# ouyangjiahong/representation-disentanglement

Measured on AMD Instinct MI355X. Metric: MR slices/sec (train step, recon+adv+latent losses), higher is better.
Workload: dtype f32

## Files before the change

### include/mrdis.h

```cpp
#ifndef MRDIS_H
#define MRDIS_H

#include <stddef.h>
#include <stdint.h>

#ifdef __cplusplus
extern "C" {
#endif

#define MRDIS_OK            0
#define MRDIS_EINVAL       -1
#define MRDIS_EUNSUPPORTED -2
#define MRDIS_EWORKSPACE   -3
#define MRDIS_ELAUNCH      -4
#define MRDIS_EALIGN       -5

#define MRDIS_MAX_TAPS 16

#define MRDIS_EPI_NONE   0
#define MRDIS_EPI_LRELU  1

const char* mrdis_strerror(int code);
int mrdis_version(void);

// ... 110 lines not shown
                                 void* dx, int lddx, void* dgamma, int lddg, void* dbeta, int lddb,
                                 void* workspace, size_t workspace_bytes,
                                 int N, int Hi, int Wi, int C, const void* xlo, int ldxlo, int dtype, void* stream);

int mrdis_bilinear_fwd(const void* x, int ldx, void* y, int ldy, int N, int Hi, int Wi,
                       int Ho, int Wo, int C, int align_corners, int dtype, void* stream);
size_t mrdis_bilinear_up2_stats_workspace(int N, int Hi, int C);
int mrdis_bilinear_up2_stats_applies(int N, int Wi, int C);
int mrdis_bilinear_up2_stats_fwd(const void* x, int ldx, void* y, int ldy, int N, int Hi, int Wi, int C,
                                 int out_block, long long out_block_stride,
                                 float* save_mean, float* save_rstd, float eps, void* workspace, size_t workspace_bytes,
                                 int dtype, void* stream);
int mrdis_bilinear_bwd(const void* dy, int lddy, void* dx, int lddx, int N, int Hi, int Wi,
                       int Ho, int Wo, int C, int align_corners, int dtype, void* stream);

int mrdis_softmax_mask_drop_fwd(const float* s, int lds, const float* mask_img, float* out, int ldo,
                                long long P, int C, float mask_scale, void* stream);
int mrdis_softmax_mask_drop_bwd(const float* dout, int lddo, const float* out, int ldo,
                                float* ds, int ldds, long long P, int C, void* stream);

size_t mrdis_recon_err_workspace(int N, long long HW, int C);
int mrdis_recon_err_fwd(const float* gt, int ldgt, const float* x, int ldx, float* out,
                        void* workspace, size_t workspace_bytes,
                        int N, long long HW, int C, int p, void* stream);
int mrdis_recon_err_bwd(const float* gt, int ldgt, const float* x, int ldx, const float* w,
                        float* dx, int lddx, int N, long long HW, int C, int p, void* stream);

size_t mrdis_recon_metrics_workspace(int n_img, int H);
int mrdis_recon_metrics(const float* target, int ldt, const float* pred, int ldp, float* out,
                        void* workspace, size_t workspace_bytes, int n_img, int H, int W, void* stream);
// ... 146 lines not shown
```

### representation-disentanglement_amd/csrc/mrdis_common.h

```cpp
#pragma once
#include <hip/hip_runtime.h>
#include <stdint.h>
#include "../../include/mrdis.h"
#include "mrdis_device.h"

#define MRDIS_CHECK_LAUNCH()                                     \
    do {                                                         \
        hipError_t e_ = hipGetLastError();                       \
        if (e_ != hipSuccess) return MRDIS_ELAUNCH;              \
    } while (0)

#define MRDIS_OPTIONS(X) \
    X(WINO, "wino", "MRDIS_WINO", 0, 1)  \
    X(NT_MB, "nt_mb", "MRDIS_NT_MB", 0, 128)  \
    X(WINO_PIPE, "wino_pipe", "MRDIS_WINO_PIPE", 0, 1)  \
    X(WINO_U, "wino_u", "MRDIS_WINO_U", 0, 1)  \
    X(WINO4, "wino4", "MRDIS_WINO4", 0, 1)  \
    X(WINO4R, "wino4r", "MRDIS_WINO4R", 0, 1)  \
    X(BCONV4, "bconv4", "MRDIS_BCONV4", 0, 1)  \
    X(SPLIT6, "split6", "MRDIS_SPLIT6", 0, 1)  \
    X(NO16, "debug_no16", "MRDIS_DEBUG_NO16", 1, 0) \
    X(NOTHIN, "debug_nothin", "MRDIS_DEBUG_NOTHIN", 1, 0) \
    X(NOC4, "debug_noc4", "MRDIS_DEBUG_NOC4", 1, 0) \
    X(NODMA, "debug_nodma", "MRDIS_DEBUG_NODMA", 1, 0) \
// ... 28 lines not shown
    X(CHATT, "chatt") X(SYMDIFF, "symdiff") X(RGATE, "rgate")  \
    X(DIRECT3D, "direct3d") X(C3D16, "c3d16") X(WGRAD3D, "wgrad3d") X(WGRAD3D16, "wgrad3d16") X(WINO_WGRAD3D, "wino_wgrad3d")  \
    X(VOLGATHER, "volgather")  \
    X(LOSS3D, "loss3d") X(SEGCOUNTS, "segcounts")  \
    X(SEGACCUM, "segaccum") X(SEGLABELS, "seglabels")  \
    X(SYNTHACCUM, "synthaccum") X(SYNTHFINISH, "synthfinish")  \
    X(SEG2DLABELS, "seg2dlabels") X(SEG2DFINISH, "seg2dfinish")  \
    X(FUSE, "fuse")  \
    X(REGSURF, "regsurf") X(EDT, "edt") X(SURFHIST, "surfhist")  \
    X(CCLABEL, "cclabel") X(CCCLEAN, "ccclean")  \
    X(STAT_VEC, "stat_vec") X(STAT_SCALAR, "stat_scalar") X(STAT_INTERP, "stat_interp")  \
    X(SPADE_UP2_ONEPASS, "spade_up2_onepass") X(SPADE_UP2_TWOPASS, "spade_up2_twopass")  \
    X(BIL_FWD_X2, "bil_fwd_x2") X(BIL_FWD_GENERAL, "bil_fwd_general")  \
    X(BIL_BWD_X2, "bil_bwd_x2") X(BIL_BWD_TIGHT3, "bil_bwd_tight3") X(BIL_BWD_TIGHT5, "bil_bwd_tight5") X(BIL_BWD_GENERAL, "bil_bwd_general")  \
    X(ELEM_V1, "elem_v1")  \
    X(ALL, "all")
#define MRDIS_X_CNT_ID(id, name) MRDIS_CNT_##id,
enum { MRDIS_COUNTERS(MRDIS_X_CNT_ID) MRDIS_CNT_COUNT };
void mrdis_count(int id);

void mrdis_note_lds(const char* kernel_expr, size_t bytes);
#define MRDIS_LAUNCH(kernel, grid, block, lds, s, ...) do { mrdis_count(MRDIS_CNT_ALL); if ((size_t)(lds) != 0) mrdis_note_lds(#kernel, (size_t)(lds)); hipLaunchKernelGGL(kernel, grid, block, lds, s, __VA_ARGS__); } while (0)

int mrdis_cu_count();
bool mrdis_lds_optin(const void* kernel, int bytes);
int mrdis_occupancy(const void* kernel, int block, size_t lds);

static inline int mrdis_cdiv(long long a, long long b) { return (int)((a + b - 1) / b); }

__device__ __forceinline__ int mrdis_xcd_remap(int bid, int nblk) {
// ... 19 lines not shown
```

### representation-disentanglement_amd/csrc/mrdis_elem.hip

```cpp
#include "mrdis_common.h"
#include <type_traits>
#include <stdlib.h>

template <int V> struct Vec;
template <> struct Vec<1> {
    float v[1];
    __device__ __forceinline__ void load(const float* p) { v[0] = p[0]; }
    __device__ __forceinline__ void store(float* p) const { p[0] = v[0]; }
    __device__ __forceinline__ void load(const __bf16* p) { v[0] = (float)p[0]; }
    __device__ __forceinline__ void store(__bf16* p) const { p[0] = (__bf16)v[0]; }
};
template <> struct Vec<4> {
    float v[4];
    __device__ __forceinline__ void load(const float* p) {
        const float4 t = *reinterpret_cast<const float4*>(p); v[0] = t.x; v[1] = t.y; v[2] = t.z; v[3] = t.w;
    }
    __device__ __forceinline__ void store(float* p) const { *reinterpret_cast<float4*>(p) = make_float4(v[0], v[1], v[2], v[3]); }
    __device__ __forceinline__ void load(const __bf16* p) {
        const bf16x4 t = *reinterpret_cast<const bf16x4*>(p); v[0] = (float)t[0]; v[1] = (float)t[1]; v[2] = (float)t[2]; v[3] = (float)t[3];
    }
    __device__ __forceinline__ void store(__bf16* p) const {
        bf16x4 t; t[0] = (__bf16)v[0]; t[1] = (__bf16)v[1]; t[2] = (__bf16)v[2]; t[3] = (__bf16)v[3];
        *reinterpret_cast<bf16x4*>(p) = t;
    }
// ... 1120 lines not shown
        MRDIS_LAUNCH((bilinear_bwd_tight_kernel<4, 3, 3, T>), dim3(Hi, N), dim3(bil_threads((long long)Wi * (C / 4))), 0, s, dy, lddy, dx, lddx, N, Hi, Wi, Ho, Wo, C, align_corners, sh, sw);
    } else if (vec4_ok(dy, lddy, C) && vec4_ok(dx, lddx, C) && tight5) {
        mrdis_count(MRDIS_CNT_BIL_BWD_TIGHT5);
        MRDIS_LAUNCH((bilinear_bwd_tight_kernel<4, 5, 5, T>), dim3(Hi, N), dim3(bil_threads((long long)Wi * (C / 4))), 0, s, dy, lddy, dx, lddx, N, Hi, Wi, Ho, Wo, C, align_corners, sh, sw);
    } else if (vec4_ok(dy, lddy, C) && vec4_ok(dx, lddx, C)) {
        mrdis_count(MRDIS_CNT_BIL_BWD_GENERAL);
        MRDIS_LAUNCH((bilinear_bwd_kernel<4, T>), dim3(Hi, N), dim3(bil_threads((long long)Wi * (C / 4))), 0, s, dy, lddy, dx, lddx, N, Hi, Wi, Ho, Wo, C, align_corners, sh, sw);
    } else {
        mrdis_count(MRDIS_CNT_BIL_BWD_GENERAL); mrdis_count(MRDIS_CNT_ELEM_V1);
        MRDIS_LAUNCH((bilinear_bwd_kernel<1, T>), dim3(Hi, N), dim3(bil_threads((long long)Wi * C)), 0, s, dy, lddy, dx, lddx, N, Hi, Wi, Ho, Wo, C, align_corners, sh, sw);
    }
    MRDIS_CHECK_LAUNCH();
    return MRDIS_OK;
}

extern "C" size_t mrdis_bilinear_up2_stats_workspace(int N, int Hi, int C) { return sizeof(float) * 2 * (size_t)N * Hi * C + 64; }
template <typename T>
static int bilinear_up2_stats_impl(const T* x, int ldx, T* y, int ldy, int N, int Hi, int Wi, int C, int out_block, long long out_block_stride,
                                   float* save_mean, float* save_rstd, float eps, void* workspace, size_t workspace_bytes, void* stream) {
    if (!x || !y || !save_mean || !save_rstd || !workspace || N < 1 || Hi < 1 || Wi < 1 || C < 1 || ldx < C || ldy < C) return MRDIS_EINVAL;
    if (out_block <= 0 || out_block >= N) { out_block = 0x7fffffff; out_block_stride = 0; }
    else if (N % out_block != 0 || out_block_stride < 4LL * out_block * Hi * Wi * ldy || out_block_stride % 4 != 0) return MRDIS_EINVAL;
    if (workspace_bytes < mrdis_bilinear_up2_stats_workspace(N, Hi, C)) return MRDIS_EWORKSPACE;
    const int threads = bil_threads((long long)Wi * (C / 4));
    if (N > 65535 || C % 4 != 0 || !vec4_ok(x, ldx, C) || !vec4_ok(y, ldy, C) || threads % (C / 4) != 0) return MRDIS_EUNSUPPORTED;
    hipStream_t s = (hipStream_t)stream;
    float* part = reinterpret_cast<float*>(workspace);
    MRDIS_LAUNCH((bilinear_up2_fwd_kernel<T, true>), dim3(Hi, N), dim3(threads), 0, s, x, ldx, y, ldy, Hi, Wi, C, part, out_block, out_block_stride);
    MRDIS_CHECK_LAUNCH();
    MRDIS_LAUNCH((stat_final_kernel<0>), dim3(mrdis_cdiv(N * C, 64)), dim3(64, stat_final_lanes(Hi)), 0, s, part, Hi, C, N, 4LL * Hi * Wi, eps, 0.f,
// ... 70 lines not shown
                          lrelu_bwd_impl((cbf)dy, lddy, (cbf)y, ldy, (bf)dx, lddx, P, C, slope, stream));
}
extern "C" int mrdis_bilinear_fwd(const void* x, int ldx, void* y, int ldy, int N, int Hi, int Wi, int Ho, int Wo, int C, int align_corners, int dtype, void* stream) {
    return MRDIS_BY_DTYPE(dtype, bilinear_fwd_impl((const float*)x, ldx, (float*)y, ldy, N, Hi, Wi, Ho, Wo, C, align_corners, stream),
                          bilinear_fwd_impl((cbf)x, ldx, (bf)y, ldy, N, Hi, Wi, Ho, Wo, C, align_corners, stream));
}
extern "C" int mrdis_bilinear_up2_stats_fwd(const void* x, int ldx, void* y, int ldy, int N, int Hi, int Wi, int C, int out_block, long long out_block_stride,
                                            float* save_mean, float* save_rstd, float eps, void* workspace, size_t workspace_bytes, int dtype, void* stream) {
    return MRDIS_BY_DTYPE(dtype,
        bilinear_up2_stats_impl((const float*)x, ldx, (float*)y, ldy, N, Hi, Wi, C, out_block, out_block_stride, save_mean, save_rstd, eps, workspace, workspace_bytes, stream),
        bilinear_up2_stats_impl((cbf)x, ldx, (bf)y, ldy, N, Hi, Wi, C, out_block, out_block_stride, save_mean, save_rstd, eps, workspace, workspace_bytes, stream));
}
extern "C" int mrdis_bilinear_bwd(const void* dy, int lddy, void* dx, int lddx, int N, int Hi, int Wi, int Ho, int Wo, int C, int align_corners, int dtype, void* stream) {
    return MRDIS_BY_DTYPE(dtype, bilinear_bwd_impl((const float*)dy, lddy, (float*)dx, lddx, N, Hi, Wi, Ho, Wo, C, align_corners, stream),
                          bilinear_bwd_impl((cbf)dy, lddy, (bf)dx, lddx, N, Hi, Wi, Ho, Wo, C, align_corners, stream));
}

template <int V, typename TS, typename TD>
__global__ void cast_view_kernel(const TS* __restrict__ src, int lds_, int Cs, TD* __restrict__ dst, int ldd, int Cd, long long P) {
    const int Q = Cd / V;
    EW_LOOP(P * Q) {
        const long long r = idx / Q; const int c = (int)(idx - r * Q) * V;
        Vec<V> a;
        if (c + V <= Cs) a.load(src + r * lds_ + c);
        else {
#pragma unroll
            for (int k = 0; k < V; ++k) a.v[k] = (c + k < Cs) ? mrdis_ld1(src + r * lds_ + c + k) : 0.f;
        }
        a.store(dst + r * ldd + c);
    }
// ... 499 lines not shown
```

### representation-disentanglement_amd/hip.py

```python
import collections
import ctypes
import os

import torch

_HERE = os.path.dirname(os.path.abspath(__file__))
LIB_PATH = os.path.join(_HERE, 'csrc', 'libmrdis_hip.so')


class MrdisLibraryError(RuntimeError):
    pass


class MrdisError(RuntimeError):
    pass


_lib = None
_c = ctypes
_P, _I, _L, _F, _Z = _c.c_void_p, _c.c_int, _c.c_longlong, _c.c_float, _c.c_size_t

_SIGS = {
    'mrdis_strerror': (_c.c_char_p, [_I]),
    'mrdis_version': (_I, []),
# ... 32 lines not shown
    'mrdis_cast_view': (_I, [_P, _I, _I, _I, _P, _I, _I, _I, _L, _P]),
    'mrdis_conv2d_bwd_weight_workspace': (_Z, [_I] * 9),
    'mrdis_conv2d_bwd_weight': (_I, [_P, _I, _P, _I, _P, _P, _P, _Z] + [_I] * 11 + [_P]),
    'mrdis_lrelu_bwd': (_I, [_P, _I, _P, _I, _P, _I, _L, _I, _F, _I, _P]),
    'mrdis_norm_workspace': (_Z, [_I, _L, _I]),
    'mrdis_bn_train_fwd': (_I, [_P, _I, _P, _I, _P, _P, _P, _P, _P, _P, _P, _Z, _L, _I, _F, _F, _I, _I, _P]),
    'mrdis_bn_eval_fwd': (_I, [_P, _I, _P, _I, _P, _P, _P, _P, _L, _I, _F, _I, _P]),
    'mrdis_bn_train_bwd': (_I, [_P, _I, _P, _I, _P, _P, _P, _P, _I, _P, _P, _P, _P, _P, _Z, _L, _I, _I, _I, _P]),
    'mrdis_instnorm_spade_fwd': (_I, [_P, _I, _P, _I, _P, _I, _P, _I, _P, _P, _P, _Z, _I, _L, _I, _F, _I, _P]),
    'mrdis_instnorm_spade_bwd_workspace': (_Z, [_I, _L, _I]),
    'mrdis_instnorm_spade_bwd': (_I, [_P, _I, _P, _I, _P, _I, _P, _P, _P, _I, _P, _I, _P, _I, _P, _Z, _I, _L, _I, _I, _P]),
    'mrdis_instnorm_spade_bwd_up2_workspace': (_Z, [_I, _I, _I, _I, _I]),
    'mrdis_instnorm_spade_bwd_up2': (_I, [_P, _I, _P, _I, _P, _I, _P, _P, _P, _I, _P, _I, _P, _I, _P, _Z, _I, _I, _I, _I, _P, _I, _I, _P]),
    'mrdis_bilinear_fwd': (_I, [_P, _I, _P, _I] + [_I] * 8 + [_P]),
    'mrdis_bilinear_bwd': (_I, [_P, _I, _P, _I] + [_I] * 8 + [_P]),
    'mrdis_bilinear_up2_stats_workspace': (_Z, [_I, _I, _I]),
    'mrdis_bilinear_up2_stats_applies': (_I, [_I, _I, _I]),
    'mrdis_bilinear_up2_stats_fwd': (_I, [_P, _I, _P, _I, _I, _I, _I, _I, _I, _L, _P, _P, _F, _P, _Z, _I, _P]),
    'mrdis_softmax_mask_drop_fwd': (_I, [_P, _I, _P, _P, _I, _L, _I, _F, _P]),
    'mrdis_softmax_mask_drop_bwd': (_I, [_P, _I, _P, _I, _P, _I, _L, _I, _P]),
    'mrdis_recon_err_workspace': (_Z, [_I, _L, _I]),
    'mrdis_recon_err_fwd': (_I, [_P, _I, _P, _I, _P, _P, _Z, _I, _L, _I, _I, _P]),
    'mrdis_recon_err_bwd': (_I, [_P, _I, _P, _I, _P, _P, _I, _I, _L, _I, _I, _P]),
    'mrdis_recon_metrics_workspace': (_Z, [_I, _I]),
    'mrdis_recon_metrics': (_I, [_P, _I, _P, _I, _P, _P, _Z, _I, _I, _I, _P]),
    'mrdis_slice_gather': (_I, [_P, _P, _P, _P, _I, _P, _P, _I, _I, _I, _I, _I, _I, _P]),
    'mrdis_volume_gather': (_I, [_P, _I, _P, _P, _I, _I, _I, _I, _I, _I, _I, _I, _I, _I, _P]),
    'mrdis_nvnet_loss_workspace': (_Z, [_L, _L]),
    'mrdis_nvnet_loss_fwd': (_I, [_P, _P, _P, _P, _P, _I, _P, _P, _P, _P, _P, _I, _c.c_double, _P, _P, _P, _Z, _P]),
    'mrdis_nvnet_loss_bwd': (_I, [_P, _P, _P, _P, _P, _I, _P, _P, _P, _P, _P, _I, _c.c_double, _P, _P, _P, _P, _P]),
# ... 104 lines not shown
                                   'zsearch')
VARIANT_FAMILIES = ('conv2src', 'ana_act')
LATENT_FAMILIES = ('kl', 'avgpool')
OUTDEC_FAMILIES = ('chatt', 'symdiff', 'rgate')
CONV3D_FAMILIES = ('direct3d', 'c3d16', 'wgrad3d', 'wgrad3d16', 'wino_wgrad3d')
DATA_FAMILIES = ('volgather',)
LOSS3D_FAMILIES = ('loss3d', 'segcounts')
SEGVOL_FAMILIES = ('segaccum', 'seglabels')
SYNTH_FAMILIES = ('synthaccum', 'synthfinish')
SEG2D_FAMILIES = ('seg2dlabels', 'seg2dfinish')
FUSE_FAMILIES = ('fuse',)
SURFDIST_FAMILIES = ('regsurf', 'edt', 'surfhist')
CC_FAMILIES = ('cclabel', 'ccclean')
ELEM_FAMILIES = ('stat_vec', 'stat_scalar', 'stat_interp', 'spade_up2_onepass', 'spade_up2_twopass', 'bil_fwd_x2', 'bil_fwd_general',
                 'bil_bwd_x2', 'bil_bwd_tight3', 'bil_bwd_tight5', 'bil_bwd_general', 'elem_v1')
SYNTH_MAX_SRC = 8
SEG2D_MAX_SETS = 16
SEG2D_MAX_VIEWS = 2
SEG2D_FLIPS = {'': 0, 'h': 1, 'w': 2}
FUSE_MAX_SRC = 8
FUSE_METHODS = ('mean', 'max', 'mean-max-min')
EDT_FAR = 1 << 30
EDT_MAX_SRC = 8
EDT_MAX_EXTENT = 1024
SURF_MAX_REGIONS = 4
CC_MAX_EXTENT = 1024
CC_LABEL_LAUNCHES = 3
CC_CONNECTIVITIES = (6, 18, 26)


# ... 7 lines not shown
    import re
    buf = _c.create_string_buffer(16384)
    load().mrdis_dynamic_lds_table(buf, 16384)
    out = {}
    for line in buf.value.decode().splitlines():
        expr, _, b = line.rpartition('=')
        if not expr or not b.isdigit():
            continue
        name = re.sub(r'<.*', '', expr.strip().lstrip('(')).strip()
        out[name] = max(out.get(name, 0), int(b))
    return out


def launch_counts(reset=False, elem=False):
    lib = load()
    fams = WINO_FAMILIES + VARIANT_FAMILIES + LATENT_FAMILIES + OUTDEC_FAMILIES + CONV3D_FAMILIES + DATA_FAMILIES + LOSS3D_FAMILIES + SEGVOL_FAMILIES + SYNTH_FAMILIES + SEG2D_FAMILIES + FUSE_FAMILIES + SURFDIST_FAMILIES + CC_FAMILIES
    out ={f: int(lib.mrdis_launch_count(f.encode())) for f in fams + (ELEM_FAMILIES if elem else ())}
    if reset:
        lib.mrdis_launch_count_reset()
    return out


class option:

    def __init__(self, name, value):
        self.name, self.value = name, value

    def __enter__(self):
        self.prev = get_option(self.name)
        set_option(self.name, self.value)

# ... 714 lines not shown

def bilinear_bwd(dy, in_hw, align_corners, out=None):
    lib = load()
    dy, lddy = nhwc(dy)
    N, C, Ho, Wo = dy.shape
    Hi, Wi = in_hw
    if out is None:
        dx = empty_nhwc(N, C, Hi, Wi, dy.device, dy.dtype)
    else:
        dx, ldo = nhwc(out)
        assert dx.data_ptr() == out.data_ptr() and ldo == C and tuple(out.shape) == (N, C, Hi, Wi) and out.dtype == dy.dtype
    _chk(lib.mrdis_bilinear_bwd(_ptr(dy), lddy, _ptr(dx), C, N, Hi, Wi, Ho, Wo, C, 1 if align_corners else 0, _dt(dy), _stream()), 'bilinear_bwd')
    return dx


def softmax_mask_drop_fwd(s, mask_img, scale=100.0):
    lib = load()
    s, lds = nhwc(s)
    N, C, H, W = s.shape
    out = empty_nhwc(N, C, H, W, s.device)
    m = None if mask_img is None else mask_img.contiguous()
    _chk(lib.mrdis_softmax_mask_drop_fwd(_ptr(s), lds, _ptr(m), _ptr(out), C, N * H * W, C, scale, _stream()), 'softmax_mask_drop_fwd')
    return out


def softmax_mask_drop_bwd(dout, out):
    lib = load()
    dout, lddo = nhwc(dout); out, ldo = nhwc(out)
    N, C, H, W = out.shape
    ds = empty_nhwc(N, C, H, W, out.device)
# ... 898 lines not shown
```

### representation-disentanglement_amd/model.py

```python
import copy
import weakref

import numpy as np
import torch
import torch.nn as nn
import torch.nn.functional as F

from . import ops


def _pair(v):
    return (v, v) if isinstance(v, int) else tuple(v)


class _routing(nn.Module):

    def __init__(self, in_channels, num_experts):
        super().__init__()
        self.fc = nn.Linear(in_channels, num_experts)

    def forward(self, inputs_type):
        return torch.sigmoid(self.fc(inputs_type))


# ... 212 lines not shown
        return self.act(x)


class Act_Deconv_BN_Concat_New(nn.Module):

    def __init__(self, in_num_ch, out_num_ch, filter_size=3, stride=1, padding=1, activation='relu', upsample=True,
                 is_last=False, is_bn=True, is_cond=False):
        super().__init__()
        if not upsample:
            raise NotImplementedError('ConvTranspose2d variant is not on the path (model.py:2178)')
        self.is_bn, self.is_cond, self.is_last = is_bn, is_cond, is_last
        self.act = nn.ELU(inplace=True) if activation == 'elu' else nn.Sequential()
        self.conv = Conv2d(is_cond)(in_num_ch, out_num_ch, filter_size, stride, padding=padding)
        self.bn = BatchNorm2d(out_num_ch)

    def forward(self, x_down, x_up, inputs_type=None):
        x_up = self.act(x_up)
        x_up = ops.bilinear(x_up, (2 * x_up.shape[2], 2 * x_up.shape[3]), True)
        x_up = self.conv(x_up, inputs_type) if self.is_cond else self.conv(x_up)
        if self.is_last:
            return x_up
        if self.is_bn and self.training and x_up.is_cuda and ops.cat_elision() and x_down.dtype == x_up.dtype and isinstance(self.act, nn.Sequential) \
                and x_down.shape[0] == x_up.shape[0] and x_down.shape[2:] == x_up.shape[2:]:
            Cd, Cu = x_down.shape[1], x_up.shape[1]
            buf = getattr(x_down, '_mrdis_catbuf', None)
            if buf is not None and buf.shape[1] == Cd + Cu and buf.dtype == x_up.dtype:
                x_down._mrdis_catbuf = None
                x_up = self.bn(x_up, into=(buf, Cd))
                return ops.cat_join(x_down, x_up, buf)
        if self.is_bn:
            x_up = self.bn(x_up)
        return torch.cat([x_down, x_up], 1)


    def forward_grouped(self, x_down, x_up, types):
        G = len(types)
        x_up = self.act(x_up)
        x_up = ops.bilinear(x_up, (2 * x_up.shape[2], 2 * x_up.shape[3]), True)
        x_up = self.conv.forward_grouped(x_up, types)
        if self.is_last:
            return x_up
        if self.is_bn and self.training and x_up.is_cuda and ops.cat_elision() and x_down.dtype == x_up.dtype and isinstance(self.act, nn.Sequential) \
                and x_down.shape[0] == x_up.shape[0] and x_down.shape[2:] == x_up.shape[2:]:
            Cd, Cu = x_down.shape[1], x_up.shape[1]
            buf = getattr(x_down, '_mrdis_catbuf', None)
            if buf is not None and buf.shape[1] == Cd + Cu and buf.dtype == x_up.dtype:
                x_down._mrdis_catbuf = None
                x_up = self.bn(x_up, into=(buf, Cd), groups=G)
                return ops.cat_join(x_down, x_up, buf)
        if self.is_bn:
            x_up = self.bn(x_up, groups=G)
        return torch.cat([x_down, x_up], 1)
# ... 1132 lines not shown
```

### representation-disentanglement_amd/ops.py

```python
import contextlib
import numpy as _np
import os as _os

import torch
from torch.autograd import Function

from . import hip


class _MixExperts(Function):

    @staticmethod
    def forward(ctx, W, r):
        w_tck, w_tkc = hip.mix_experts_fwd(W, r)
        ctx.save_for_backward(W, r)
        ctx.mark_non_differentiable(w_tkc)
        return w_tck, w_tkc

    @staticmethod
    def backward(ctx, g_tck, _g_tkc):
        W, r = ctx.saved_tensors
        dW, dr = hip.mix_experts_bwd(g_tck, W, r)
        return dW, dr

# ... 970 lines not shown
    @staticmethod
    def forward(ctx, x, out_hw, align_corners):
        ctx.geom = (x.shape[2], x.shape[3], align_corners)
        return hip.bilinear_fwd(x, out_hw, align_corners)

    @staticmethod
    def backward(ctx, dy):
        Hi, Wi, ac = ctx.geom
        return hip.bilinear_bwd(dy, (Hi, Wi), ac), None, None


def bilinear(x, out_hw, align_corners):
    return _Bilinear.apply(x, tuple(out_hw), bool(align_corners))


class _BilinearUp2Stats(Function):

    @staticmethod
    def forward(ctx, x, eps):
        ctx.geom = (x.shape[2], x.shape[3])
        res = hip.bilinear_up2_stats(x, eps)
        if res is None:
            y = hip.bilinear_fwd(x, (2 * x.shape[2], 2 * x.shape[3]), False)
            mean = rstd = torch.empty(0, dtype=torch.float32, device=x.device)
        else:
            y, mean, rstd = res
        ctx.mark_non_differentiable(mean, rstd)
        return y, mean, rstd

    @staticmethod
# ... 749 lines not shown
```

Before: 253.3.

## Fold final 3x3 conv before bilinear upsample via 1x1 conv and tap-sum kernel

```diff
diff --git a/include/mrdis.h b/include/mrdis.h
--- a/include/mrdis.h
+++ b/include/mrdis.h
@@ -148,6 +148,11 @@
 int mrdis_bilinear_bwd(const void* dy, int lddy, void* dx, int lddx, int N, int Hi, int Wi,
                        int Ho, int Wo, int C, int align_corners, int dtype, void* stream);
 
+int mrdis_up2_tapsum_fwd(const float* M, int ldm, const float* bias, float* y, int ldy, int N, int h, int w, int Co, void* stream);
+size_t mrdis_up2_tapsum_bwd_workspace(int N, int h, int w, int Co);
+int mrdis_up2_tapsum_bwd(const float* dy, int lddy, float* G, int ldg, float* dbias, int accumulate_bias, void* workspace, size_t workspace_bytes,
+                         int N, int h, int w, int Co, void* stream);
+
 int mrdis_softmax_mask_drop_fwd(const float* s, int lds, const float* mask_img, float* out, int ldo,
                                 long long P, int C, float mask_scale, void* stream);
 int mrdis_softmax_mask_drop_bwd(const float* dout, int lddo, const float* out, int ldo,
diff --git a/representation-disentanglement_amd/csrc/mrdis_common.h b/representation-disentanglement_amd/csrc/mrdis_common.h
--- a/representation-disentanglement_amd/csrc/mrdis_common.h
+++ b/representation-disentanglement_amd/csrc/mrdis_common.h
@@ -66,6 +66,7 @@
     X(BIL_FWD_X2, "bil_fwd_x2") X(BIL_FWD_GENERAL, "bil_fwd_general")  \
     X(BIL_BWD_X2, "bil_bwd_x2") X(BIL_BWD_TIGHT3, "bil_bwd_tight3") X(BIL_BWD_TIGHT5, "bil_bwd_tight5") X(BIL_BWD_GENERAL, "bil_bwd_general")  \
     X(ELEM_V1, "elem_v1")  \
+    X(UP2TAPSUM, "up2tapsum")  \
     X(ALL, "all")
 #define MRDIS_X_CNT_ID(id, name) MRDIS_CNT_##id,
 enum { MRDIS_COUNTERS(MRDIS_X_CNT_ID) MRDIS_CNT_COUNT };
diff --git a/representation-disentanglement_amd/csrc/mrdis_elem.hip b/representation-disentanglement_amd/csrc/mrdis_elem.hip
--- a/representation-disentanglement_amd/csrc/mrdis_elem.hip
+++ b/representation-disentanglement_amd/csrc/mrdis_elem.hip
@@ -1158,6 +1158,306 @@
     return MRDIS_OK;
 }
 
+constexpr int HEAD_TH = 16, HEAD_TW = 64, HEAD_LH = HEAD_TH / 2 + 3, HEAD_LW = HEAD_TW / 2 + 3;
+template <int CO>
+__device__ __forceinline__ void head_lds_load(const float* p, float (&v)[CO]) {
+    if constexpr (CO == 4) { const float4 t = *reinterpret_cast<const float4*>(p); v[0] = t.x; v[1] = t.y; v[2] = t.z; v[3] = t.w; }
+    else {
+#pragma unroll
+        for (int o = 0; o < CO; ++o) v[o] = p[o];
+    }
+}
+template <int CO>
+__device__ __forceinline__ void head_lds_store(float* p, const float (&v)[CO]) {
+    if constexpr (CO == 4) *reinterpret_cast<float4*>(p) = make_float4(v[0], v[1], v[2], v[3]);
+    else {
+#pragma unroll
+        for (int o = 0; o < CO; ++o) p[o] = v[o];
+    }
+}
+template <int CO>
+__global__ __launch_bounds__(256) void up2_tapsum_fwd_kernel(const float* __restrict__ M, int ldm, const float* __restrict__ bias, float* __restrict__ y, int ldy,
+                                                             int h, int w, float sh, float sw, int vec_m, int vec_y) {
+    constexpr int C9 = 9 * CO;
+    extern __shared__ __attribute__((aligned(16))) float head_tile[];
+    const int Ho = 2 * h, Wo = 2 * w, n = blockIdx.z;
+    const int Y0 = blockIdx.y * HEAD_TH, X0 = blockIdx.x * HEAD_TW;
+    const int ya = Y0 > 0 ? Y0 - 1 : 0, yb = Y0 + HEAD_TH < Ho ? Y0 + HEAD_TH : Ho - 1;
+    const int xa = X0 > 0 ? X0 - 1 : 0, xb = X0 + HEAD_TW < Wo ? X0 + HEAD_TW : Wo - 1;
+    const int r0 = bil_axis(ya, sh, 1, h).i0, c0 = bil_axis(xa, sw, 1, w).i0;
+    int nr = bil_axis(yb, sh, 1, h).i1 - r0 + 1, nc = bil_axis(xb, sw, 1, w).i1 - c0 + 1;
+    if (nr > HEAD_LH) nr = HEAD_LH;
+    if (nc > HEAD_LW) nc = HEAD_LW;
+    const float* src = M + (((long long)n * h + r0) * w + c0) * ldm;
+    if (CO == 4 && vec_m) {
+        constexpr int Q = C9 / 4, RPW = (HEAD_LH + 3) / 4, IPR = (HEAD_LW * Q + 63) / 64;
+        const int wave = threadIdx.x >> 6, lane = threadIdx.x & 63;
+        float4 t[RPW][IPR];
+#pragma unroll
+        for (int a = 0; a < RPW; ++a)
+#pragma unroll
+            for (int k = 0; k < IPR; ++k) {
+                const int r = wave + 4 * a, it = lane + 64 * k;
+                const bool ok = r < nr && it < nc * Q;
+                const int rc = ok ? r : 0, pix = (ok ? it : 0) / Q, q = (ok ? it : 0) - pix * Q;
+                t[a][k] = mrdis_ld4(src + ((long long)rc * w + pix) * ldm + 4 * q);
+            }
+#pragma unroll
+        for (int a = 0; a < RPW; ++a)
+#pragma unroll
+            for (int k = 0; k < IPR; ++k) {
+                const int r = wave + 4 * a, it = lane + 64 * k;
+                if (r < nr && it < nc * Q) *reinterpret_cast<float4*>(head_tile + r * (HEAD_LW * C9) + 4 * it) = t[a][k];
+            }
+    } else {
+        for (int idx = threadIdx.x; idx < nr * nc * C9; idx += 256) {
+            const int pix = idx / C9, k = idx - pix * C9, r = pix / nc, c = pix - r * nc;
+            head_tile[(r * HEAD_LW + c) * C9 + k] = src[((long long)r * w + c) * ldm + k];
+        }
+    }
+    __syncthreads();
+    float b[CO];
+#pragma unroll
+    for (int o = 0; o < CO; ++o) b[o] = bias ? bias[o] : 0.f;
+    for (int p = threadIdx.x; p < HEAD_TH * HEAD_TW; p += 256) {
+        const int Y = Y0 + p / HEAD_TW, X = X0 + p % HEAD_TW;
+        if (Y >= Ho || X >= Wo) continue;
+        BilAxis ah[3], aw[3];
+        bool vh[3], vw[3];
+#pragma unroll
+        for (int k = 0; k < 3; ++k) {
+            const int yy = Y + k - 1, xx = X + k - 1;
+            vh[k] = yy >= 0 && yy < Ho; vw[k] = xx >= 0 && xx < Wo;
+            ah[k] = bil_axis(vh[k] ? yy : Y, sh, 1, h); aw[k] = bil_axis(vw[k] ? xx : X, sw, 1, w);
+            ah[k].i0 = min(ah[k].i0 - r0, HEAD_LH - 1) * (HEAD_LW * C9); ah[k].i1 = min(ah[k].i1 - r0, HEAD_LH - 1) * (HEAD_LW * C9);
+            aw[k].i0 = min(aw[k].i0 - c0, HEAD_LW - 1) * C9; aw[k].i1 = min(aw[k].i1 - c0, HEAD_LW - 1) * C9;
+        }
+        float acc[CO];
+#pragma unroll
+        for (int o = 0; o < CO; ++o) acc[o] = b[o];
+#pragma unroll
+        for (int kh = 0; kh < 3; ++kh)
+#pragma unroll
+            for (int kw = 0; kw < 3; ++kw) {
+                if (!(vh[kh] && vw[kw])) continue;
+                const float* t = head_tile + (kh * 3 + kw) * CO;
+                float p00[CO], p01[CO], p10[CO], p11[CO];
+                head_lds_load<CO>(t + ah[kh].i0 + aw[kw].i0, p00); head_lds_load<CO>(t + ah[kh].i0 + aw[kw].i1, p01);
+                head_lds_load<CO>(t + ah[kh].i1 + aw[kw].i0, p10); head_lds_load<CO>(t + ah[kh].i1 + aw[kw].i1, p11);
+#pragma unroll
+                for (int o = 0; o < CO; ++o)
+                    acc[o] += ah[kh].l0 * (aw[kw].l0 * p00[o] + aw[kw].l1 * p01[o]) + ah[kh].l1 * (aw[kw].l0 * p10[o] + aw[kw].l1 * p11[o]);
+            }
+        float* yo = y + (((long long)n * Ho + Y) * Wo + X) * ldy;
+        if (CO == 4 && vec_y) mrdis_st4(yo, make_float4(acc[0], acc[CO > 1 ? 1 : 0], acc[CO > 2 ? 2 : 0], acc[CO > 3 ? 3 : 0]));
+        else {
+#pragma unroll
+            for (int o = 0; o < CO; ++o) yo[o] = acc[o];
+        }
+    }
+}
+
+constexpr int HEADB_LH = 8, HEADB_LW = 32, HEADB_NA = 6;
+constexpr int HEADB_DH = 2 * HEADB_LH + HEADB_NA + 4, HEADB_DW = 2 * HEADB_LW + HEADB_NA + 4;
+__device__ __forceinline__ float bil_adj_weight(int o, int i, float scale, int isz) {
+    const BilAxis a = bil_axis(o, scale, 1, isz);
+    return (a.i0 == i ? a.l0 : 0.f) + (a.i1 == i ? a.l1 : 0.f);
+}
+__device__ __forceinline__ int bil_adj_first(int i, float scale, int isz, int osz, int* last) {
+    int lo, hi;
+    bil_range(i, scale, 1, osz, &lo, &hi);
+    while (lo < hi && bil_adj_weight(lo, i, scale, isz) == 0.f) ++lo;
+    *last = hi;
+    return lo;
+}
+template <int CO>
+__global__ __launch_bounds__(256) void up2_tapsum_bwd_kernel(const float* __restrict__ dy, int lddy, float* __restrict__ G, int ldg, double* __restrict__ dbpart,
+                                                             int h, int w, float sh, float sw, int vec_dy, int vec_g) {
+    constexpr int C9 = 9 * CO;
+    extern __shared__ __attribute__((aligned(16))) float head_tile[];
+    const int Ho = 2 * h, Wo = 2 * w, n = blockIdx.z;
+    const int i0t = blockIdx.y * HEADB_LH, j0t = blockIdx.x * HEADB_LW;
+    const int ilast = min(i0t + HEADB_LH, h) - 1, jlast = min(j0t + HEADB_LW, w) - 1;
+    int unused;
+    const auto uni = [](int v) { return __builtin_amdgcn_readfirstlane(v); };
+    const int R0 = uni(bil_adj_first(i0t, sh, h, Ho, &unused) - 1), C0 = uni(bil_adj_first(j0t, sw, w, Wo, &unused) - 1);
+    const int needH = uni(min(bil_adj_first(ilast, sh, h, Ho, &unused) + HEADB_NA + 1 - R0, HEADB_DH));
+    const int needW = uni(min(bil_adj_first(jlast, sw, w, Wo, &unused) + HEADB_NA + 1 - C0, HEADB_DW));
+    const int oR0 = blockIdx.y == 0 ? 0 : R0, oC0 = blockIdx.x == 0 ? 0 : C0;
+    const int oR1 = blockIdx.y + 1 == gridDim.y ? Ho : uni(bil_adj_first(i0t + HEADB_LH, sh, h, Ho, &unused) - 1);
+    const int oC1 = blockIdx.x + 1 == gridDim.x ? Wo : uni(bil_adj_first(j0t + HEADB_LW, sw, w, Wo, &unused) - 1);
+    const float* base = dy + (long long)n * Ho * Wo * lddy;
+    double dbs[CO];
+#pragma unroll
+    for (int o = 0; o < CO; ++o) dbs[o] = 0.0;
+    constexpr int NST = (HEADB_DH * HEADB_DW + 255) / 256;
+    float v[NST][CO];
+#pragma unroll
+    for (int k = 0; k < NST; ++k) {
+        const int idx = threadIdx.x + 256 * k, r = idx / HEADB_DW, c = idx - r * HEADB_DW;
+        const int Rc = min(max(R0 + r, 0), Ho - 1), Cc = min(max(C0 + c, 0), Wo - 1);
+        const float* p = base + ((long long)Rc * Wo + Cc) * lddy;
+        if (CO == 4 && vec_dy) { const float4 t = mrdis_ld4(p); v[k][0] = t.x; v[k][CO > 1 ? 1 : 0] = t.y; v[k][CO > 2 ? 2 : 0] = t.z; v[k][CO > 3 ? 3 : 0] = t.w; }
+        else {
+#pragma unroll
+            for (int o = 0; o < CO; ++o) v[k][o] = p[o];
+        }
+    }
+#pragma unroll
+    for (int k = 0; k < NST; ++k) {
+        const int idx = threadIdx.x + 256 * k, r = idx / HEADB_DW, c = idx - r * HEADB_DW, R = R0 + r, C = C0 + c;
+        const bool in = r < needH && c < needW && R >= 0 && R < Ho && C >= 0 && C < Wo;
+        const bool own = in && R >= oR0 && R < oR1 && C >= oC0 && C < oC1;
+#pragma unroll
+        for (int o = 0; o < CO; ++o) {
+            v[k][o] = in ? v[k][o] : 0.f;
+            dbs[o] += own ? (double)v[k][o] : 0.0;
+        }
+        if (idx < HEADB_DH * HEADB_DW) head_lds_store<CO>(head_tile + idx * CO, v[k]);
+    }
+    __syncthreads();
+    const int ty = threadIdx.x / HEADB_LW, tx = threadIdx.x % HEADB_LW;
+    const int i = min(i0t + ty, h - 1), j = min(j0t + tx, w - 1);
+    int hhi, whi;
+    const int hs = bil_adj_first(i, sh, h, Ho, &hhi), ws = bil_adj_first(j, sw, w, Wo, &whi);
+    float whv[HEADB_NA], wwv[HEADB_NA];
+#pragma unroll
+    for (int a = 0; a < HEADB_NA; ++a) {
+        whv[a] = hs + a <= hhi ? bil_adj_weight(hs + a, i, sh, h) : 0.f;
+        wwv[a] = ws + a <= whi ? bil_adj_weight(ws + a, j, sw, w) : 0.f;
+    }
+    const int rr0 = hs - 1 - R0, cc0 = ws - 1 - C0;
+    float acc[9][CO];
+#pragma unroll
+    for (int t = 0; t < 9; ++t)
+#pragma unroll
+        for (int o = 0; o < CO; ++o) acc[t][o] = 0.f;
+#pragma unroll
+    for (int r = 0; r < HEADB_NA + 2; ++r) {
+        const float* row = head_tile + min(rr0 + r, HEADB_DH - 1) * (HEADB_DW * CO);
+        float v[HEADB_NA + 2][CO];
+#pragma unroll
+        for (int q = 0; q < HEADB_NA + 2; ++q) {
+            head_lds_load<CO>(row + min(cc0 + q, HEADB_DW - 1) * CO, v[q]);
+        }
+#pragma unroll
+        for (int kw = 0; kw < 3; ++kw) {
+            float c3[CO];
+#pragma unroll
+            for (int o = 0; o < CO; ++o) c3[o] = 0.f;
+#pragma unroll
+            for (int bq = 0; bq < HEADB_NA; ++bq)
+#pragma unroll
+                for (int o = 0; o < CO; ++o) c3[o] += wwv[bq] * v[bq + 2 - kw][o];
+#pragma unroll
+            for (int kh = 0; kh < 3; ++kh) {
+                const int a = r + kh - 2;
+                if (a < 0 || a >= HEADB_NA) continue;
+#pragma unroll
+                for (int o = 0; o < CO; ++o) acc[kh * 3 + kw][o] += whv[a] * c3[o];
+            }
+        }
+#pragma unroll
+        for (int t = 0; t < 9; ++t)
+#pragma unroll
+            for (int o = 0; o < CO; ++o) asm volatile("" : "+v"(acc[t][o]));
+    }
+    __syncthreads();
+    if (dbpart) {
+#pragma unroll
+        for (int o = 0; o < CO; ++o) dbs[o] = mrdis_wave_sum_d(dbs[o]);
+    }
+#pragma unroll
+    for (int t = 0; t < 9; ++t) head_lds_store<CO>(head_tile + threadIdx.x * C9 + t * CO, acc[t]);
+    double* wsum = reinterpret_cast<double*>(head_tile + 256 * C9);
+    if (dbpart && (threadIdx.x & 63) == 0) {
+#pragma unroll
+        for (int o = 0; o < CO; ++o) wsum[(threadIdx.x >> 6) * CO + o] = dbs[o];
+    }
+    __syncthreads();
+    if (dbpart && threadIdx.x < CO) {
+        const long long wg = ((long long)blockIdx.z * gridDim.y + blockIdx.y) * gridDim.x + blockIdx.x;
+        dbpart[wg * CO + threadIdx.x] = ((wsum[threadIdx.x] + wsum[CO + threadIdx.x]) + wsum[2 * CO + threadIdx.x]) + wsum[3 * CO + threadIdx.x];
+    }
+    const int nrow = ilast - i0t + 1, ncol = jlast - j0t + 1;
+    float* gout = G + (((long long)n * h + i0t) * w + j0t) * ldg;
+    if (CO == 4 && vec_g) {
+        constexpr int Q = C9 / 4;
+        for (int idx = threadIdx.x; idx < nrow * ncol * Q; idx += 256) {
+            const int pix = idx / Q, q = idx - pix * Q, r = pix / ncol, c = pix - r * ncol;
+            mrdis_st4(gout + ((long long)r * w + c) * ldg + 4 * q, *reinterpret_cast<const float4*>(head_tile + (r * HEADB_LW + c) * C9 + 4 * q));
+        }
+    } else {
+        for (int idx = threadIdx.x; idx < nrow * ncol * C9; idx += 256) {
+            const int pix = idx / C9, k = idx - pix * C9, r = pix / ncol, c = pix - r * ncol;
+            gout[((long long)r * w + c) * ldg + k] = head_tile[(r * HEADB_LW + c) * C9 + k];
+        }
+    }
+}
+__global__ __launch_bounds__(256) void up2_tapsum_dbias_kernel(const double* __restrict__ part, long long nparts, int Co, float* __restrict__ dbias, int accumulate) {
+    __shared__ double red[4];
+    for (int o = 0; o < Co; ++o) {
+        double s = 0.0;
+        for (long long k = threadIdx.x; k < nparts; k += 256) s += part[k * Co + o];
+        s = mrdis_wave_sum_d(s);
+        if ((threadIdx.x & 63) == 0) red[threadIdx.x >> 6] = s;
+        __syncthreads();
+        if (threadIdx.x == 0) {
+            const float t = (float)(((red[0] + red[1]) + red[2]) + red[3]);
+            dbias[o] = accumulate ? dbias[o] + t : t;
+        }
+        __syncthreads();
+    }
+}
+
+static inline bool head_geom_ok(int N, int h, int w, int Co) { return N >= 1 && N <= 65535 && h >= 1 && w >= 1 && h <= (1 << 20) && w <= (1 << 20) && Co >= 1 && Co <= 4; }
+static inline bool head_al16(const float* p, int ld) { return ld % 4 == 0 && ((uintptr_t)p & 15) == 0; }
+
+static int up2_tapsum_fwd_impl(const float* M, int ldm, const float* bias, float* y, int ldy, int N, int h, int w, int Co, hipStream_t s) {
+    if (!M || !y || !head_geom_ok(N, h, w, Co) || ldm < 9 * Co || ldy < Co) return MRDIS_EINVAL;
+    const dim3 grid(mrdis_cdiv(2 * w, HEAD_TW), mrdis_cdiv(2 * h, HEAD_TH), N);
+    if (grid.y > 65535) return MRDIS_EUNSUPPORTED;
+    const size_t lds = sizeof(float) * HEAD_LH * HEAD_LW * 9 * Co;
+    const float sh = bil_scale(h, 2 * h, 1), sw = bil_scale(w, 2 * w, 1);
+    const int vm = head_al16(M, ldm), vy = head_al16(y, ldy);
+    mrdis_count(MRDIS_CNT_UP2TAPSUM);
+#define HEAD_FWD(co) { if (!mrdis_lds_optin((const void*)up2_tapsum_fwd_kernel<co>, 64 * 1024)) return MRDIS_ELAUNCH; \
+                       MRDIS_LAUNCH((up2_tapsum_fwd_kernel<co>), grid, dim3(256), lds, s, M, ldm, bias, y, ldy, h, w, sh, sw, vm, vy); }
+    if (Co == 4) HEAD_FWD(4) else if (Co == 3) HEAD_FWD(3) else if (Co == 2) HEAD_FWD(2) else HEAD_FWD(1)
+#undef HEAD_FWD
+    MRDIS_CHECK_LAUNCH();
+    return MRDIS_OK;
+}
+static inline long long head_bwd_parts(int N, int h, int w) { return (long long)N * mrdis_cdiv(h, HEADB_LH) * mrdis_cdiv(w, HEADB_LW); }
+static int up2_tapsum_bwd_impl(const float* dy, int lddy, float* G, int ldg, float* dbias, int accumulate_bias, void* workspace, size_t workspace_bytes,
+                               int N, int h, int w, int Co, hipStream_t s) {
+    if (!dy || !G || !head_geom_ok(N, h, w, Co) || lddy < Co || ldg < 9 * Co) return MRDIS_EINVAL;
+    const dim3 grid(mrdis_cdiv(w, HEADB_LW), mrdis_cdiv(h, HEADB_LH), N);
+    if (grid.y > 65535) return MRDIS_EUNSUPPORTED;
+    const long long nparts = head_bwd_parts(N, h, w);
+    double* part = nullptr;
+    if (dbias) {
+        if (!workspace || workspace_bytes < sizeof(double) * nparts * Co) return MRDIS_EWORKSPACE;
+        if (((uintptr_t)workspace & 7) != 0) return MRDIS_EALIGN;
+        part = reinterpret_cast<double*>(workspace);
+    }
+    const size_t tile = sizeof(float) * HEADB_DH * HEADB_DW * Co, outb = sizeof(float) * 256 * 9 * Co + sizeof(double) * 4 * Co;
+    const size_t lds = tile > outb ? tile : outb;
+    const float sh = bil_scale(h, 2 * h, 1), sw = bil_scale(w, 2 * w, 1);
+    const int vd = head_al16(dy, lddy), vg = head_al16(G, ldg);
+    mrdis_count(MRDIS_CNT_UP2TAPSUM);
+#define HEAD_BWD(co) { if (!mrdis_lds_optin((const void*)up2_tapsum_bwd_kernel<co>, 64 * 1024)) return MRDIS_ELAUNCH; \
+                       MRDIS_LAUNCH((up2_tapsum_bwd_kernel<co>), grid, dim3(256), lds, s, dy, lddy, G, ldg, part, h, w, sh, sw, vd, vg); }
+    if (Co == 4) HEAD_BWD(4) else if (Co == 3) HEAD_BWD(3) else if (Co == 2) HEAD_BWD(2) else HEAD_BWD(1)
+#undef HEAD_BWD
+    MRDIS_CHECK_LAUNCH();
+    if (dbias) {
+        MRDIS_LAUNCH(up2_tapsum_dbias_kernel, dim3(1), dim3(256), 0, s, part, nparts, Co, dbias, accumulate_bias ? 1 : 0);
+        MRDIS_CHECK_LAUNCH();
+    }
+    return MRDIS_OK;
+}
+
 extern "C" size_t mrdis_bilinear_up2_stats_workspace(int N, int Hi, int C) { return sizeof(float) * 2 * (size_t)N * Hi * C + 64; }
 template <typename T>
 static int bilinear_up2_stats_impl(const T* x, int ldx, T* y, int ldy, int N, int Hi, int Wi, int C, int out_block, long long out_block_stride,
@@ -1258,6 +1558,16 @@
 extern "C" int mrdis_bilinear_bwd(const void* dy, int lddy, void* dx, int lddx, int N, int Hi, int Wi, int Ho, int Wo, int C, int align_corners, int dtype, void* stream) {
     return MRDIS_BY_DTYPE(dtype, bilinear_bwd_impl((const float*)dy, lddy, (float*)dx, lddx, N, Hi, Wi, Ho, Wo, C, align_corners, stream),
                           bilinear_bwd_impl((cbf)dy, lddy, (bf)dx, lddx, N, Hi, Wi, Ho, Wo, C, align_corners, stream));
+}
+extern "C" int mrdis_up2_tapsum_fwd(const float* M, int ldm, const float* bias, float* y, int ldy, int N, int h, int w, int Co, void* stream) {
+    return up2_tapsum_fwd_impl(M, ldm, bias, y, ldy, N, h, w, Co, (hipStream_t)stream);
+}
+extern "C" size_t mrdis_up2_tapsum_bwd_workspace(int N, int h, int w, int Co) {
+    return head_geom_ok(N, h, w, Co) ? sizeof(double) * (size_t)head_bwd_parts(N, h, w) * Co + 64 : 0;
+}
+extern "C" int mrdis_up2_tapsum_bwd(const float* dy, int lddy, float* G, int ldg, float* dbias, int accumulate_bias, void* workspace, size_t workspace_bytes,
+                                    int N, int h, int w, int Co, void* stream) {
+    return up2_tapsum_bwd_impl(dy, lddy, G, ldg, dbias, accumulate_bias, workspace, workspace_bytes, N, h, w, Co, (hipStream_t)stream);
 }
 
 template <int V, typename TS, typename TD>
diff --git a/representation-disentanglement_amd/hip.py b/representation-disentanglement_amd/hip.py
--- a/representation-disentanglement_amd/hip.py
+++ b/representation-disentanglement_amd/hip.py
@@ -70,6 +70,9 @@
     'mrdis_instnorm_spade_bwd_up2': (_I, [_P, _I, _P, _I, _P, _I, _P, _P, _P, _I, _P, _I, _P, _I, _P, _Z, _I, _I, _I, _I, _P, _I, _I, _P]),
     'mrdis_bilinear_fwd': (_I, [_P, _I, _P, _I] + [_I] * 8 + [_P]),
     'mrdis_bilinear_bwd': (_I, [_P, _I, _P, _I] + [_I] * 8 + [_P]),
+    'mrdis_up2_tapsum_fwd': (_I, [_P, _I, _P, _P, _I, _I, _I, _I, _I, _P]),
+    'mrdis_up2_tapsum_bwd_workspace': (_Z, [_I, _I, _I, _I]),
+    'mrdis_up2_tapsum_bwd': (_I, [_P, _I, _P, _I, _P, _I, _P, _Z, _I, _I, _I, _I, _P]),
     'mrdis_bilinear_up2_stats_workspace': (_Z, [_I, _I, _I]),
     'mrdis_bilinear_up2_stats_applies': (_I, [_I, _I, _I]),
     'mrdis_bilinear_up2_stats_fwd': (_I, [_P, _I, _P, _I, _I, _I, _I, _I, _I, _L, _P, _P, _F, _P, _Z, _I, _P]),
@@ -204,6 +207,7 @@
 CC_FAMILIES = ('cclabel', 'ccclean')
 ELEM_FAMILIES = ('stat_vec', 'stat_scalar', 'stat_interp', 'spade_up2_onepass', 'spade_up2_twopass', 'bil_fwd_x2', 'bil_fwd_general',
                  'bil_bwd_x2', 'bil_bwd_tight3', 'bil_bwd_tight5', 'bil_bwd_general', 'elem_v1')
+HEAD_FAMILIES = ('up2tapsum',)
 SYNTH_MAX_SRC = 8
 SEG2D_MAX_SETS = 16
 SEG2D_MAX_VIEWS = 2
@@ -241,7 +245,7 @@
 
 def launch_counts(reset=False, elem=False):
     lib = load()
-    fams = WINO_FAMILIES + VARIANT_FAMILIES + LATENT_FAMILIES + OUTDEC_FAMILIES + CONV3D_FAMILIES + DATA_FAMILIES + LOSS3D_FAMILIES + SEGVOL_FAMILIES + SYNTH_FAMILIES + SEG2D_FAMILIES + FUSE_FAMILIES + SURFDIST_FAMILIES + CC_FAMILIES
+    fams = WINO_FAMILIES + VARIANT_FAMILIES + LATENT_FAMILIES + OUTDEC_FAMILIES + CONV3D_FAMILIES + DATA_FAMILIES + LOSS3D_FAMILIES + SEGVOL_FAMILIES + SYNTH_FAMILIES + SEG2D_FAMILIES + FUSE_FAMILIES + SURFDIST_FAMILIES + CC_FAMILIES + HEAD_FAMILIES
     out ={f: int(lib.mrdis_launch_count(f.encode())) for f in fams + (ELEM_FAMILIES if elem else ())}
     if reset:
         lib.mrdis_launch_count_reset()
@@ -986,6 +990,47 @@
     return dx
 
 
+HEAD_MAX_CO = 4
+
+
+def up2_tapsum_applies(N, Co):
+    return 1 <= Co <= HEAD_MAX_CO and 1 <= N <= 65535
+
+
+def up2_tapsum_fwd(M, bias, Co, out=None):
+    lib = load()
+    M, ldm = nhwc(M)
+    N, C9, h, w = M.shape
+    assert C9 == 9 * Co and M.dtype is torch.float32, (M.shape, Co, M.dtype)
+    if out is None:
+        out = empty_nhwc(N, Co, 2 * h, 2 * w, M.device)
+    y, ldy = nhwc(out)
+    assert y.data_ptr() == out.data_ptr() and tuple(out.shape) == (N, Co, 2 * h, 2 * w) and out.dtype is torch.float32
+    _chk(lib.mrdis_up2_tapsum_fwd(_ptr(M), ldm, _ptr(bias), _ptr(y), ldy, N, h, w, Co, _stream()), 'up2_tapsum_fwd')
+    return out
+
+
+def up2_tapsum_bwd(dy, need_bias=True, bias_sink=None, out=None):
+    lib = load()
+    dy, lddy = nhwc(dy)
+    N, Co, Ho, Wo = dy.shape
+    assert Ho % 2 == 0 and Wo % 2 == 0 and dy.dtype is torch.float32, (dy.shape, dy.dtype)
+    h, w = Ho // 2, Wo // 2
+    if out is None:
+        out = empty_nhwc(N, 9 * Co, h, w, dy.device)
+    G, ldg = nhwc(out)
+    assert G.data_ptr() == out.data_ptr() and tuple(out.shape) == (N, 9 * Co, h, w) and out.dtype is torch.float32
+    sink = bias_sink if need_bias else None
+    db = torch.empty(Co, dtype=torch.float32, device=dy.device) if (need_bias and sink is None) else None
+    ws, nb = None, 0
+    if need_bias:
+        nb = _ws_bytes(lib.mrdis_up2_tapsum_bwd_workspace, N, h, w, Co)
+        ws = _ws(nb, dy.device)
+    _chk(lib.mrdis_up2_tapsum_bwd(_ptr(dy), lddy, _ptr(G), ldg, _ptr(sink if sink is not None else db), 1 if sink is not None else 0,
+                                  _ptr(ws), nb, N, h, w, Co, _stream()), 'up2_tapsum_bwd')
+    return out, db
+
+
 def softmax_mask_drop_fwd(s, mask_img, scale=100.0):
     lib = load()
     s, lds = nhwc(s)
diff --git a/representation-disentanglement_amd/model.py b/representation-disentanglement_amd/model.py
--- a/representation-disentanglement_amd/model.py
+++ b/representation-disentanglement_amd/model.py
@@ -250,8 +250,25 @@
         self.conv = Conv2d(is_cond)(in_num_ch, out_num_ch, filter_size, stride, padding=padding)
         self.bn = BatchNorm2d(out_num_ch)
 
+    def _head_filter(self, x_up, inputs_type):
+        c = self.conv
+        if not (c.kernel_size == (3, 3) and c.stride == (1, 1) and c.padding == (1, 1) and ops.head_fold_applies(x_up, c.in_channels, c.out_channels)):
+            return None
+        if self.is_cond:
+            if not (x_up.shape[0] == 1 or inputs_type.stride(0) == 0):
+                return None
+            return c.mixed_uniform(inputs_type)
+        if c.dilation != (1, 1) or c.groups != 1 or c.padding_mode != 'zeros':
+            return None
+        one = torch.ones(1, dtype=torch.float32, device=x_up.device)
+        return ops.cached_mix((id(c), 0, 0), lambda: ops.mix_experts(c.weight.unsqueeze(0), one))
+
     def forward(self, x_down, x_up, inputs_type=None):
         x_up = self.act(x_up)
+        if self.is_last:
+            filt = self._head_filter(x_up, inputs_type)
+            if filt is not None:
+                return ops.conv3x3_after_up2(x_up, filt[0], filt[1], self.conv.bias)
         x_up = ops.bilinear(x_up, (2 * x_up.shape[2], 2 * x_up.shape[3]), True)
         x_up = self.conv(x_up, inputs_type) if self.is_cond else self.conv(x_up)
         if self.is_last:
@@ -272,6 +289,11 @@
     def forward_grouped(self, x_down, x_up, types):
         G = len(types)
         x_up = self.act(x_up)
+        if self.is_last and self.is_cond and x_up.shape[0] % G == 0:
+            filts = [self._head_filter(x_up, t) for t in types]
+            if all(f is not None for f in filts):
+                blocks = ops.split_batch(x_up, G)
+                return torch.cat([ops.conv3x3_after_up2(blocks[g], filts[g][0], filts[g][1], self.conv.bias) for g in range(G)], 0)
         x_up = ops.bilinear(x_up, (2 * x_up.shape[2], 2 * x_up.shape[3]), True)
         x_up = self.conv.forward_grouped(x_up, types)
         if self.is_last:
diff --git a/representation-disentanglement_amd/ops.py b/representation-disentanglement_amd/ops.py
--- a/representation-disentanglement_amd/ops.py
+++ b/representation-disentanglement_amd/ops.py
@@ -1008,6 +1008,50 @@
     return _Bilinear.apply(x, tuple(out_hw), bool(align_corners))
 
 
+_HEAD_FOLD = _os.environ.get('MRDIS_HEAD_FOLD', '1') != '0'
+
+
+def set_head_fold(enabled):
+    global _HEAD_FOLD
+    _HEAD_FOLD = bool(enabled)
+
+
+class _Up2TapSum(Function):
+
+    @staticmethod
+    def forward(ctx, M, bias, Co):
+        ctx.bias_param = bias
+        return hip.up2_tapsum_fwd(M, bias, Co)
+
+    @staticmethod
+    def backward(ctx, dy):
+        bias = ctx.bias_param
+        need_b = bias is not None and ctx.needs_input_grad[1]
+        sink = _grad_sink(bias) if need_b else None
+        G, db = hip.up2_tapsum_bwd(dy, need_bias=need_b, bias_sink=sink)
+        return G, db, None
+
+
+def up2_tapsum(M, bias, Co):
+    return _Up2TapSum.apply(M, bias, int(Co))
+
+
+def head_fold_applies(x, Ci, Co):
+    return (_HEAD_FOLD and _COMPUTE_DTYPE == hip.DT_F32 and _MIX_CACHE is not None and torch.is_grad_enabled() and type(x) is torch.Tensor
+            and x.is_cuda and x.dtype is torch.float32 and x.dim() == 4 and x.shape[1] == Ci and hip.up2_tapsum_applies(x.shape[0], Co))
+
+
+def conv3x3_after_up2(x, w_tck, w_tkc, bias):
+    T, Ci, Co = w_tck.shape
+    assert T == 9 and tuple(w_tkc.shape) == (9, Co, Ci), (w_tck.shape, w_tkc.shape)
+
+    def regroup():
+        return (w_tck, w_tck.permute(1, 0, 2).reshape(1, Ci, 9 * Co), w_tkc.reshape(1, 9 * Co, Ci))
+    _, w1_tck, w1_tkc = cached_mix(('head1x1', id(w_tck)), regroup)
+    M = conv2d(x, w1_tck, w1_tkc, None, 1, 1, 1, 0)
+    return up2_tapsum(M, bias, Co)
+
+
 class _BilinearUp2Stats(Function):
 
     @staticmethod
```

After: 201.3. 0.795x the previous value.
